# SunJiamei/LRP-ImageCaptioning

Measured on AMD Instinct MI355X. Metric: LRP heatmaps/sec (per predicted token) VGG16+adaptive-attn, 224x224, higher is better.
Workload: dtype bf16x3; 1 GPU; batch=32 synthetic 224x224 per GPU, VGG16 + adaptive-attention, LRP per-token heat-maps, 10 words/caption, V=10000 (BASELINE configs[1]); parallelism=image-sharded x1, RCCL weight broadcast, reverse_walk_precision=bf16x3, handles_per_gpu=2

## Files before the change

include/lrp_hip.h:

```cpp
#ifndef LRP_HIP_H
#define LRP_HIP_H

#include <stddef.h>
#include <stdint.h>

#ifdef __cplusplus
extern "C" {
#endif

#define LRP_ABI_VERSION 10

enum {
  LRP_OK = 0,
  LRP_ERR_INVALID = -1,
  LRP_ERR_STATE = -2,
  LRP_ERR_HIP = -3,
  LRP_ERR_NOMEM = -4,
  LRP_ERR_RANGE = -5,
  LRP_ERR_UNSUPPORTED = -6
};

enum { LRP_DEC_ADAPTIVE = 0,
       LRP_DEC_GRIDTD = 1 };

// ... 148 lines not shown
                   const float* mask_logits_dev, float* grads_dev, float* losses_dev, void* stream);
int lrp_train_forward(lrp_handle* h, int32_t B, int32_t T, const int32_t* cap_in_dev, const float* mask_image_features_dev,
                      const float* mask_global_dev, const float* mask_output_dev, const float* mask_lstm_in_dev,
                      const float* mask_lstm_rec_dev, void* stream);
int lrp_train_drop_forward(lrp_handle* h, void* stream);
int lrp_train_apply(lrp_handle* h, const float* grads_dev, void* stream);
int lrp_train_get_master(lrp_handle* h, float* flat_dev, void* stream);

int64_t lrp_launch_count(void);

int lrp_reload_switches(void);

enum { LRP_EPI_BIAS_RELU = 0, LRP_EPI_BIAS = 1, LRP_EPI_MUL = 2, LRP_EPI_MUL_UP2 = 3, LRP_EPI_FWD_DUAL = 4, LRP_EPI_STORE = 5,
       LRP_EPI_IMG_STENCIL = 6 };
enum { LRP_OPND_FP32 = 0, LRP_OPND_BF16X3 = 1, LRP_OPND_F16X2 = 2 };
enum { LRP_FORM_PLAIN = 0, LRP_FORM_SMALL = 1, LRP_FORM_HALO = 2, LRP_FORM_BREG = 3, LRP_FORM_POOL = 4, LRP_FORM_IMG = 5 };
enum { LRP_PLAN_FRAG = 1, LRP_PLAN_JOIN = 2, LRP_PLAN_DUAL_IL = 4, LRP_PLAN_GMASK = 8,
       LRP_PLAN_UP2_SRC = 16, LRP_PLAN_IMG_PART = 32, LRP_PLAN_POOL_GC = 64 };
int lrp_conv_plan(int32_t epi, int32_t prec, int32_t terms, int32_t NB, int32_t H, int32_t W, int32_t N, int32_t Cin, int32_t taps,
                  int32_t split, uint32_t flags, int32_t* out11);

const char* lrp_last_error(void);
int lrp_abi_version(void);

#ifdef __cplusplus
}
#endif
#endif
```

lrp-imagecaptioning_amd/_capi.py:

```python
import ctypes as C
import os

HERE = os.path.dirname(os.path.abspath(__file__))
LIB_PATH = os.path.join(HERE, "liblrp_hip.so")

LRP_ABI_VERSION = 10
LRP_OK, LRP_ERR_INVALID, LRP_ERR_STATE, LRP_ERR_HIP, LRP_ERR_NOMEM, LRP_ERR_RANGE, LRP_ERR_UNSUPPORTED = 0, -1, -2, -3, -4, -5, -6
LRP_DEC_ADAPTIVE, LRP_DEC_GRIDTD = 0, 1
LRP_ENC_VGG, LRP_ENC_RESNET = 0, 1
LRP_EXPLAIN_SEQUENCE, LRP_EXPLAIN_SINGLE_STEP = 0, 1
LRP_PREC_FP32, LRP_PREC_BF16X3, LRP_PREC_BF16X3_FAST, LRP_PREC_F16X2 = 0, 1, 2, 3
LRP_MAX_CONV = 32
LRP_TRAIN_FP32, LRP_TRAIN_BF16 = 0, 1
LRP_EPI_BIAS_RELU, LRP_EPI_BIAS, LRP_EPI_MUL, LRP_EPI_MUL_UP2, LRP_EPI_FWD_DUAL, LRP_EPI_STORE, LRP_EPI_IMG_STENCIL = range(7)
LRP_OPND_FP32, LRP_OPND_BF16X3, LRP_OPND_F16X2 = 0, 1, 2
LRP_FORM_PLAIN, LRP_FORM_SMALL, LRP_FORM_HALO, LRP_FORM_BREG, LRP_FORM_POOL, LRP_FORM_IMG = range(6)
LRP_PLAN_FRAG, LRP_PLAN_JOIN, LRP_PLAN_DUAL_IL, LRP_PLAN_GMASK, LRP_PLAN_UP2_SRC, LRP_PLAN_IMG_PART, LRP_PLAN_POOL_GC = 1, 2, 4, 8, 16, 32, 64


class LrpConfig(C.Structure):
    _fields_ = [
        ("abi_version", C.c_int32), ("device", C.c_int32), ("decoder", C.c_int32),
        ("img_h", C.c_int32), ("img_w", C.c_int32), ("n_conv", C.c_int32),
        ("conv_cin", C.c_int32 * LRP_MAX_CONV), ("conv_cout", C.c_int32 * LRP_MAX_CONV),
        ("conv_pool_after", C.c_int32 * LRP_MAX_CONV), ("conv_name", (C.c_char * 32) * LRP_MAX_CONV),
        ("L", C.c_int32), ("D", C.c_int32), ("H", C.c_int32), ("E", C.c_int32), ("V", C.c_int32),
        ("max_images", C.c_int32), ("max_tokens", C.c_int32), ("max_caption_len", C.c_int32),
        ("sos_id", C.c_int32), ("eos_id", C.c_int32),
        ("encoder", C.c_int32), ("resnet_stem", C.c_int32), ("resnet_n_stacks", C.c_int32),
        ("resnet_filters", C.c_int32 * 8), ("resnet_blocks", C.c_int32 * 8),
    ]
# ... 102 lines not shown
```

lrp-imagecaptioning_amd/csrc/cnn_kernels.h:

```cpp
#pragma once
#include <hip/hip_runtime.h>
#include "conv_igemm.h"

namespace lrp {

__device__ __forceinline__ float safe_den(float z) { return z + (z == 0.f ? 1e-7f : 0.f); }

__global__ __launch_bounds__(256) void im2col_image_kernel(const float* __restrict__ img, float* __restrict__ A1,
                                                           int NB, int H, int W) {
  const size_t idx = (size_t)blockIdx.x * 256 + threadIdx.x;
  const size_t total = (size_t)NB * H * W * 8;
  if (idx >= total) return;
  const int g = (int)(idx & 7);
  const size_t m = idx >> 3;
  const int HW = H * W;
  const int n = (int)(m / HW), rem = (int)(m - (size_t)n * HW);
  const int h = rem / W, w = rem - h * W;
  const bool neg = g >= 4;
  float v[8];
#pragma unroll
  for (int q = 0; q < 8; ++q) {
    const int kk = 8 * (g & 3) + q;
    float x = 0.f;
    if (kk < 27) {
// ... 390 lines not shown

__global__ __launch_bounds__(256) void pack_image_layer_dev_kernel(const float* __restrict__ w, float* __restrict__ fwd,
                                                                   float* __restrict__ bwd, float* __restrict__ full, int cout, int Kb) {
  const int i = blockIdx.x * 256 + threadIdx.x;
  if (i >= 27 * cout) return;
  const int k = i / cout, co = i - k * cout, t = k / 3, c = k - 3 * t;
  const float v = w[i], vp = v >= 0.f ? v : 0.f, vn = v < 0.f ? v : 0.f;
  fwd[(size_t)co * 64 + k] = v;
  fwd[(size_t)co * 64 + 32 + k] = v;
  fwd[(size_t)(cout + co) * 64 + k] = vp;
  fwd[(size_t)(cout + co) * 64 + 32 + k] = vn;
  bwd[(size_t)(t * 6 + c) * Kb + co] = vp;
  bwd[(size_t)(t * 6 + 3 + c) * Kb + co] = vn;
  full[(size_t)(t * 6 + c) * Kb + co] = v;
}
__global__ __launch_bounds__(256) void pack_frag64_dev_kernel(const float* __restrict__ src, float* __restrict__ dst, int CP) {
  const int K = 9 * CP, cpt = CP / 32;
  const size_t total = (size_t)cpt * 9 * 4 * 2 * 64;
  for (size_t i = (size_t)blockIdx.x * 256 + threadIdx.x; i < total; i += (size_t)gridDim.x * 256) {
    const int n = (int)(i & 63), hh = (int)((i >> 6) & 1), q = (int)((i >> 7) & 3);
    const int kc = (int)(i >> 9), cc = kc / 9, t = kc % 9;
    const int c = 4 * (q >> 1) + 2 * hh + (q & 1);
    *reinterpret_cast<f32x4*>(dst + i * 4) = *reinterpret_cast<const f32x4*>(src + (size_t)n * K + t * CP + cc * 32 + c * 4);
  }
}

__global__ __launch_bounds__(256) void top_divide_kernel(const f32x4* __restrict__ R, const f32x4* __restrict__ Ztop,
                                                         const int* __restrict__ row2img, f32x4* __restrict__ S,
                                                         int n, size_t per_img4) {
  const size_t total = (size_t)n * per_img4;
  for (size_t i = (size_t)blockIdx.x * 256 + threadIdx.x; i < total; i += (size_t)gridDim.x * 256) {
    const int t = (int)(i / per_img4);
    const size_t e = i - (size_t)t * per_img4;
    const int img = row2img ? row2img[t] : t;
    const f32x4 r = R[i], z = Ztop[(size_t)img * per_img4 + e];
    f32x4 o;
// ... 115 lines not shown
```

lrp-imagecaptioning_amd/csrc/common.h:

```cpp
#pragma once
#include <hip/hip_runtime.h>
#include <atomic>
#include <cstdarg>
#include <cstdio>
#include <cstdlib>
#include <string>
#include <vector>

#include "../../include/lrp_hip.h"

namespace lrp {

inline std::atomic<unsigned long long> g_launch_count{0};
#undef hipLaunchKernelGGL
#define hipLaunchKernelGGL(kernelName, numBlocks, numThreads, memPerBlock, streamId, ...)                  \
  do {                                                                                                    \
    ::lrp::g_launch_count.fetch_add(1, std::memory_order_relaxed);                                       \
    kernelName<<<(numBlocks), (numThreads), (memPerBlock), (streamId)>>>(__VA_ARGS__);                   \
  } while (0)

std::string& last_error_ref();

struct Switches {
  int conv_halo = 1;
  int conv_breg = 1;
  int conv_small = 1;
  int conv_mid = 1;
  int epi_fast = 1;
  int up2_pw = 1;
  int tile_order = 1;
  int fwd_emit = 1;
  int fwd_il = 1;
  int img_fused = 1;
  int up2_compact = 1;
  int img_fold = 1;
  int pool_fused = 1;
  int sparse_pool = 1;
  void load() {
    *this = Switches();
    auto rd = [](const char* name, int& v) { if (const char* e = getenv(name)) v = atoi(e); };
    rd("LRP_CONV_HALO", conv_halo); rd("LRP_CONV_BREG", conv_breg); rd("LRP_CONV_SMALL", conv_small);
    rd("LRP_CONV_MID", conv_mid); rd("LRP_EPI_FAST", epi_fast); rd("LRP_UP2_PW", up2_pw); rd("LRP_TILE_ORDER", tile_order);
    rd("LRP_FWD_EMIT", fwd_emit); rd("LRP_FWD_IL", fwd_il); rd("LRP_IMG_FUSED", img_fused); rd("LRP_UP2_COMPACT", up2_compact);
    rd("LRP_IMG_FOLD", img_fold); rd("LRP_SPARSE_POOL", sparse_pool); rd("LRP_POOL_FUSED", pool_fused);
  }
};
inline Switches& sw() {
  static Switches s = [] { Switches t; t.load(); return t; }();
  return s;
}

inline int fail(int code, const char* fmt, ...) {
  char buf[512];
  va_list ap;
  va_start(ap, fmt);
  vsnprintf(buf, sizeof(buf), fmt, ap);
  va_end(ap);
  last_error_ref() = buf;
  return code;
// ... 99 lines not shown
```

lrp-imagecaptioning_amd/csrc/conv_igemm.h:

```cpp
#pragma once
#include <hip/hip_runtime.h>
#include <stdint.h>
#include <stdlib.h>
#include <string.h>
#include <algorithm>
#include <vector>

#include "common.h"

namespace lrp {

typedef float f32x4 __attribute__((ext_vector_type(4)));
typedef float f32x16 __attribute__((ext_vector_type(16)));
typedef unsigned int u32x4 __attribute__((ext_vector_type(4)));
typedef __bf16 bf16x8 __attribute__((ext_vector_type(8)));
typedef _Float16 f16x8 __attribute__((ext_vector_type(8)));

enum ConvPrec { PREC_FP32 = 0, PREC_BF16X3 = 1, PREC_F16X2 = 2 };

__device__ __forceinline__ void split8h_store(const float* r, float* dst) {
  f16x8 hi, lo;
#pragma unroll
  for (int q = 0; q < 8; ++q) {
    hi[q] = (_Float16)r[q];
// ... 98 lines not shown
  float* pool_x;
};
constexpr int ACT_MAX_SLOTS = 64;

constexpr int LDS_STRIDE = 32;

__device__ __attribute__((aligned(16))) float lrp_zero_page[4] = {0.f, 0.f, 0.f, 0.f};

constexpr int conv_min_waves(int NW, int TM, int TN, bool halo = false) { return NW == 8 || halo ? 2 : (TM * TN >= 4 ? 2 : 3); }

constexpr int HALO_PITCH = 16, HALO_PL = 4;
constexpr int conv_halo_rows(int BM) { return BM == 256 ? 352 : 192; }

template <int WM, int WN, int TM, int TN, int EPI, int PREC, bool HALO = false, bool BREG = false, int TERMS = 7, int NS = 2,
          bool GMASK = false>
__global__ __launch_bounds__(64 * WM * WN, BREG ? 3 : NS > 2 ? 2 : conv_min_waves(WM * WN, TM, TN, HALO)) void conv_igemm_kernel(ConvArgs a) {
#if defined(__HIP_DEVICE_COMPILE__)
  constexpr int NW = WM * WN, NT = 64 * NW;
  constexpr bool SPLIT = PREC != PREC_FP32;
  constexpr int BM = WM * TM * 32, BN = WN * TN * 32;
  constexpr int AP = BM / 8 / NW, BP = BN / 8 / NW;
  constexpr int HR = conv_halo_rows(BM);
  constexpr int ABUF = (HALO ? HR : BM) * LDS_STRIDE;
  constexpr int STAGE = ABUF + (BREG ? 0 : BN) * LDS_STRIDE;
  static_assert(!BREG || (HALO && SPLIT && BM * BN <= 2 * STAGE), "BREG needs the resident image");
  static_assert((BM / 8) % NW == 0 && (BN / 8) % NW == 0, "pieces must divide over the waves");
  static_assert(!HALO || EPI != EPI_STORE, "the image layer is a 1-tap GEMM");
  static_assert(NS == 2 || (NS > 2 && !HALO && !BREG), "deeper staging exists for the plain (non-resident) A path only");
  constexpr int DPC = AP + BP;
  static_assert((NS - 2) * DPC <= 63, "vmcnt is a 6-bit counter");
  __shared__ __attribute__((aligned(16))) float smem[NS * STAGE];

  const int nblk = a.m_tiles * a.n_tiles;
  int logical;
  {
    const int bid = blockIdx.x, q = nblk >> 3, r = nblk & 7, xcd = bid & 7, idx = bid >> 3;
    logical = (xcd < r ? xcd * (q + 1) : r * (q + 1) + (xcd - r) * q) + idx;
  }
  const int mt = logical / a.n_tiles, nt = logical - mt * a.n_tiles;
  const int m0 = mt * BM, n0 = nt * BN;
  int pn = 0, py0 = 0, px0 = 0;
  if constexpr (EPI == EPI_IMG_STENCIL) {
    const int tpi = a.tiles_x * a.tiles_y;
    pn = mt / tpi;
    const int r = mt - pn * tpi, ty = r / a.tiles_x;
    py0 = ty * IMG_TILE;
// ... 30 lines not shown
        simg0 = HALO ? img0 : m0 / a.img_rows;
        simg1 = simg0 + 1 < a.n_imgs ? simg0 + 1 : simg0;
      }
      if constexpr (PREC == PREC_F16X2) { us0 = a.in_unscale[simg0]; us1 = a.in_unscale[simg1]; }
      if (a.pairs_out) { ps0 = a.pairs_scale[simg0]; ps1 = a.pairs_scale[simg1]; }
    }
  }

  const int tid = threadIdx.x, lane = tid & 63, wave = tid >> 6;
  const int wm = wave / WN, wn = wave - wm * WN;
  const int HW = a.H * a.W;
  const int K = a.taps * a.CinP;
  const int cpt = a.CinP >> 5;
  const int nk = a.taps * cpt;

  const int prow = lane >> 3, pchk = lane & 7;
  const int wave_s = __builtin_amdgcn_readfirstlane(wave);
  typedef __attribute__((address_space(3))) void* lptr_t;
  constexpr int OOB = (int)0x80000000;
  constexpr int RSRC_FLAGS = 0x00020000;
  const __amdgpu_buffer_rsrc_t rsB =
      __builtin_amdgcn_make_buffer_rsrc((void*)(a.wpk + (size_t)n0 * K), 0, BN * K * 4, RSRC_FLAGS);
  int bvo[BP];
#pragma unroll
  for (int p = 0; p < BP; ++p) {
    const int r = (wave_s * BP + p) * 8 + prow;
    bvo[p] = (r * K + ((pchk ^ ((r >> 1) & 7)) << 2)) * 4;
  }
  const float* abase = HALO ? a.in + (size_t)(Y0 > 0 ? Y0 - 1 : 0) * a.W * a.Cin
                       : EPI == EPI_IMG_STENCIL ? a.in + (size_t)pn * HW * a.Cin
                            : a.in + ((long)m0 - (a.taps == 1 ? 0 : a.W + 1)) * (long)a.Cin;
// ... 156 lines not shown
#pragma unroll
      for (int d = 0; d < 4; ++d) {
        const unsigned p0 = (w.q[d >> 1] >> (16 * (d & 1))) & 0xFFu, p1 = (w.q[d >> 1] >> (16 * (d & 1) + 8)) & 0xFFu;
        const unsigned m = r.valid ? ((p0 == j ? 0x0000FFFFu : 0u) | (p1 == j ? 0xFFFF0000u : 0u)) : 0u;
        mh[d] = w.hi[d] & m;
        ml[d] = w.lo[d] & m;
      }
      const int row = r.hy * HALO_PITCH + hx;
      const int swzu = ((r.hy * a.tw + hx - 1) >> 1) & 7;
      const int dst = abuf * STAGE + row * LDS_STRIDE + (((2 * r.g) ^ swzu) << 2);
      *reinterpret_cast<u32x4*>(smem + dst) = mh;
      *reinterpret_cast<u32x4*>(smem + (dst ^ 4)) = ml;
    }
  };
  [[maybe_unused]] PwItem pwi{};
  if constexpr (BREG) {
    if (PREC == PREC_BF16X3 && a.up2_src) {
      const int Hp = a.H >> 1, Wp = a.W >> 1;
      const int h0 = Y0 - img0 * a.H;
      const int wy0 = (h0 - 1) >> 1, wx0 = (x0 - 1) >> 1;
      const int nwx = ((x0 + a.tw) >> 1) - wx0 + 1, nwy = ((h0 + a.th) >> 1) - wy0 + 1;
      const int items = nwy * nwx * 8;
      const int ntok = img0 < a.NB ? img0 : a.NB - 1;
      const int img = a.row2img ? a.row2img[ntok] : ntok;
      const float inv_nwx = 1.0f / (float)nwx;
      constexpr int UW = 2;
      typedef unsigned u32x2_ __attribute__((ext_vector_type(2)));
      for (int it0 = tid; it0 < items; it0 += NT * UW) {
        f32x4 pv[UW][2];
        u32x2_ qv[UW];
        int wyv[UW], wxv[UW], cgv[UW];
// ... 167 lines not shown
          if constexpr ((TERMS & 2) != 0) acc[i][j] = __builtin_amdgcn_mfma_f32_32x32x16_bf16(ah, bl, acc[i][j], 0, 0, 0);
          if constexpr ((TERMS & 4) != 0) acc[i][j] = __builtin_amdgcn_mfma_f32_32x32x16_bf16(ah, bh, acc[i][j], 0, 0, 0);
        }
    } else {
#pragma unroll
      for (int s = 0; s < 4; ++s)
#pragma unroll
        for (int i = 0; i < TM; ++i)
#pragma unroll
          for (int j = 0; j < TN; ++j)
            acc[i][j] = __builtin_amdgcn_mfma_f32_32x32x2f32(__builtin_bit_cast(f32x4, f.a[i])[s],
                                                             __builtin_bit_cast(f32x4, f.b[j])[s], acc[i][j], 0, 0, 0);
    }
  };

  if constexpr (BREG) {
    static_assert(NSTEP == 2, "bf16x3");
    const __amdgpu_buffer_rsrc_t rsF = __builtin_amdgcn_make_buffer_rsrc((void*)a.wpk_frag, 0, nk * 8 * BN * 16, RSRC_FLAGS);
    const int fvo = ((lane >> 5) * BN + wn * TN * 32 + (lane & 31)) * 16;
    struct BFrag { u32x4 v[4 * TN]; };
    auto load_b = [&](BFrag& b, int kc) {
#pragma unroll
      for (int q = 0; q < 4; q += ((PREC == PREC_F16X2 && !(TERMS & 2)) ? 2 : 1))
#pragma unroll
        for (int j = 0; j < TN; ++j)
          b.v[q * TN + j] = __builtin_amdgcn_raw_buffer_load_b128(rsF, fvo + j * 32 * 16, ((kc * 4 + q) * 2) * BN * 16, 0);
    };
    struct AFrag { u32x4 v[4 * TM]; };
    auto load_a = [&](AFrag& f, const float* Ab) {
#pragma unroll
      for (int q = 0; q < 4; ++q)
// ... 288 lines not shown
        const float sc = a.tok_fac[pn];
#pragma unroll
        for (int c = 0; c < 3; ++c) { pos[c] *= sc; neg[c] *= sc; }
      }
      const float* xv = a.ximg + ((size_t)img * HW + (size_t)y * a.W + x) * 3;
      float* ov = a.out + ((size_t)pn * HW + (size_t)y * a.W + x) * 3;
#pragma unroll
      for (int c = 0; c < 3; ++c) {
        if (a.img_mode == 0) ov[c] = xv[c] >= 0.f ? xv[c] * pos[c] : xv[c] * neg[c];
        else if (a.img_mode == 1) ov[c] = pos[c] + neg[c];
        else ov[c] = xv[c] * (pos[c] + neg[c]);
      }
    }
    return;
  } else if constexpr (EPI != EPI_STORE) {
    constexpr int NH = (BM * BN + 2 * STAGE - 1) / (2 * STAGE);
    constexpr int RH = BM / NH;
    static_assert(BM % NH == 0 && RH % (TM * 32) == 0 && RH * BN <= 2 * STAGE, "slab must hold whole wave tiles");
    float* Cs = smem;
    constexpr bool SPLIT_OUT = SPLIT && (EPI == EPI_MUL || EPI == EPI_MUL_UP2);
    constexpr int CW = SPLIT_OUT ? 8 : 4;
    constexpr int C4 = BN / CW, RPP = NT / C4;
    const int c4 = tid % C4, rin = tid / C4;
    const int col = n0 + c4 * CW;
    const int tn0 = m0 / HW, tp0 = m0 - tn0 * HW;
    const float invw = 1.0f / (float)a.W;
    auto locate = [&](int lr, int& row, int& n, int& h, int& w) -> bool {
      if constexpr (HALO) {
        int ty, tx;
        divmod(lr, a.tw, inv_tw, ty, tx);
        const int Y = Y0 + ty;
        w = x0 + tx;
        if (lr >= a.th * a.tw || Y >= yend || w >= a.W) return false;
// ... 527 lines not shown
struct ConvTile { int BM, BN; };
inline ConvTile conv_pick_tile(int N) {
  if (N > 64) return {128, 128};
  if (N > 32) return {128, 64};
  return {128, 32};
}
inline int conv_npad(int N) { ConvTile t = conv_pick_tile(N); return (N + t.BN - 1) / t.BN * t.BN; }
inline int conv_cinp(int Cin) { return (Cin + 31) / 32 * 32; }

enum ConvForm {
  FORM_PLAIN = 0,
  FORM_SMALL = 1,
  FORM_HALO = 2,
  FORM_BREG = 3,
  FORM_POOL = 4,
  FORM_IMG = 5
};
struct ConvAsk {
  int epi = EPI_MUL, prec = PREC_FP32, terms = 7;
  bool gmask = false;
  int NB = 0, H = 0, W = 0, N = 0, Cin = 0, taps = 9;
  bool frag = false;
  bool join = false;
  bool dual_il = false;
  int split = 0;
  bool up2_src = false, img_part = false, pool_gc = false;
};
struct ConvPlan {
  bool ok;
  int form, BM, BN, threads;
  int M, m_tiles, n_tiles, tw, th, hrows, cols_t, nyh, tpt, epi_generic;
// ... 95 lines not shown
  const bool small = s.conv_small && t.BM == 128 && t.BN >= 64 && grid <= CONV_SMALL_BLOCKS;
  if (q.up2_src) {
    if (!mul || prec != PREC_BF16X3 || !s.up2_pw || mode <= 0 || t.BN < 128 || small || !conv_compact_shape(q.N, q.Cin, q.H, q.W))
      return refused;
  } else if (small) {
    t = {64, 64};
    p.m_tiles = (p.M + 63) / 64;
    p.n_tiles = (q.N + 63) / 64;
    return done(FORM_SMALL);
  } else if (s.conv_mid && s.conv_small && t.BM == 128 && t.BN == 128 && (q.N % 64) == 0 && grid <= 2 * CONV_SMALL_BLOCKS) {
    t = {128, 64};
    p.n_tiles = (q.N + 63) / 64;
  }
  if (mode > 0 && (t.BN >= 128 || (mode == 2 && t.BN >= 64)) && resident(false, 0.9f)) {
    if (q.up2_src && p.hrows * ((p.tw + 2) / 2 + 1) * 4 > 2 * (t.BM == 256 ? 512 : 256)) return refused;
    return done(FORM_HALO);
  }
  if (asked) return refused;
  return done(FORM_PLAIN);
}

inline const int* conv_tile_order(const ConvArgs& a, hipStream_t st) {
  if (!sw().tile_order || !a.order || !a.row2img_host || a.NB < 2 || a.th < 1) return nullptr;
  TileOrder& o = *a.order;
  const int tiles_y = a.tpt > 0 ? a.NB * a.tpt : (a.nyh + a.th - 1) / a.th;
  const bool same = o.H == a.H && o.th == a.th && o.nyh == a.nyh && o.cols_t == a.cols_t && o.tpt == a.tpt && (int)o.sig.size() == a.NB &&
                    memcmp(o.sig.data(), a.row2img_host, (size_t)a.NB * sizeof(int)) == 0;
  if (same) return o.identity ? nullptr : o.dev;
  o.sig.assign(a.row2img_host, a.row2img_host + a.NB);
  o.H = a.H; o.th = a.th; o.nyh = a.nyh; o.cols_t = a.cols_t; o.tpt = a.tpt;
// ... 81 lines not shown
inline hipError_t conv_launch_epi(ConvArgs a, hipStream_t st) {
  static_assert(!GMASK || (EPI == EPI_MUL && PREC == PREC_FP32), "byte-mask gates: exact fp32 EPI_MUL only");
  constexpr bool MUL = EPI == EPI_MUL || EPI == EPI_MUL_UP2, FWD = EPI == EPI_BIAS || EPI == EPI_BIAS_RELU || EPI == EPI_FWD_DUAL;
  if (GMASK && (a.out2s || a.gate_none)) return hipErrorInvalidValue;
  if (PREC == PREC_F16X2 && MUL && (!a.tok_fac || !a.tok_max_out || a.out_plain)) return hipErrorInvalidValue;
  if (PREC == PREC_F16X2 && FWD && !a.in_unscale) return hipErrorInvalidValue;
  const ConvPlan p = conv_plan(conv_ask(EPI, PREC, TERMS, GMASK, a));
  if (!p.ok) return hipErrorInvalidValue;
  if (p.M <= 0 || a.N <= 0) return hipSuccess;
  if (a.pool_gc && (!a.pairs_out || !a.pool_pos)) return hipErrorInvalidValue;
  if (a.img_part && !a.img_w) return hipErrorInvalidValue;
  if (a.up2_src && (!a.up2_pairs || !a.up2_gpos)) return hipErrorInvalidValue;
  conv_apply_plan(p, a);
  const dim3 grid(p.m_tiles * p.n_tiles), block(p.threads);
  if constexpr (PREC != PREC_FP32 && (MUL || FWD)) {
    if (p.form == FORM_BREG || p.form == FORM_HALO || p.form == FORM_POOL) {
      if constexpr (MUL) {
        a.tile_map = conv_tile_order(a, st);
        if (p.form == FORM_BREG) {
          hipLaunchKernelGGL((conv_igemm_kernel<2, 2, 2, 1, EPI, PREC, true, true, TERMS>), grid, block, 0, st, a);
          return hipGetLastError();
        }
      }
      if (p.BM == 256)
        hipLaunchKernelGGL((conv_igemm_kernel<2, 4, 4, 2, EPI, PREC, true, false, TERMS>), grid, block, 0, st, a);
      else if (p.BN == 128)
        hipLaunchKernelGGL((conv_igemm_kernel<2, 2, 2, 2, EPI, PREC, true, false, TERMS>), grid, block, 0, st, a);
      else
        hipLaunchKernelGGL((conv_igemm_kernel<2, 2, 2, 1, EPI, PREC, true, false, TERMS>), grid, block, 0, st, a);
      return hipGetLastError();
    }
  }
  if constexpr (PREC != PREC_FP32) {
// ... 69 lines not shown
```

lrp-imagecaptioning_amd/csrc/encoder.h:

```cpp
#pragma once
#include <algorithm>
#include <functional>
#include <memory>
#include <string>
#include <vector>

#include "cnn_kernels.h"
#include "common.h"
#include "conv_igemm.h"
#include "conv_sparse.h"
#include "f16_operand.h"
#include "fwd_mode.h"

namespace lrp {

struct ConvLayer {
  std::string name;
  int cin = 0, cout = 0, H = 0, W = 0;
  bool pool_after = false;
  bool have_w = false, have_b = false;
  DevBuf w_fwd;
  DevBuf w_fwd_a;
  DevBuf w_fwd_zs;
  DevBuf w_fwd_as;
// ... 188 lines not shown
        L.w_fwd_il.release();
      }
      LRP_TRY(mk(L.w_bwd, nb)); LRP_TRY(mk(L.w_bwd_s, nb)); LRP_TRY(mk(L.w_bwd_full, nb)); LRP_TRY(mk(L.w_bwd_h, nb));
      return LRP_OK;
    }
    const size_t Kf = (size_t)9 * conv_cinp(L.cin), Kb = (size_t)9 * conv_cinp(L.cout);
    const size_t nf = (size_t)conv_npad(L.cout) * Kf, nb = (size_t)conv_npad(L.cin) * Kb;
    LRP_TRY(mk(L.w_fwd, (size_t)conv_npad(2 * L.cout) * Kf)); LRP_TRY(mk(L.w_fwd_h, (size_t)conv_npad(2 * L.cout) * Kf));
    if (dual_interleaved(L)) LRP_TRY(mk(L.w_fwd_il, (size_t)conv_npad(2 * L.cout) * Kf));
    else L.w_fwd_il.release();
    LRP_TRY(mk(L.w_fwd_a, nf)); LRP_TRY(mk(L.w_fwd_zs, nf)); LRP_TRY(mk(L.w_fwd_as, nf));
    LRP_TRY(mk(L.w_bwd, nb)); LRP_TRY(mk(L.w_bwd_s, nb)); LRP_TRY(mk(L.w_bwd_full, nb)); LRP_TRY(mk(L.w_bwd_full_s, nb));
    LRP_TRY(mk(L.w_bwd_h, nb));
    if (L.sparse_ok() && L.idxp.p) LRP_TRY(mk(L.w_sp, conv_sparse_weight_floats(L.cin, L.cout)));
    if (conv_npad(L.cin) == 64) { LRP_TRY(mk(L.w_bwd_frag, (size_t)64 * Kb)); LRP_TRY(mk(L.w_bwd_frag_h, (size_t)64 * Kb)); }
    if (pack_tmp.bytes < nf * sizeof(float)) LRP_TRY(pack_tmp.alloc(nf * sizeof(float), total));
    return LRP_OK;
  }
  int repack_conv_weight_from_device(int li, const float* w_dev, float* tmp, hipStream_t st) {
    ConvLayer& L = layers[li];
    if (li == 0) {
      const int Npb = conv_npad(IMG_T_COLS), Kb = conv_cinp(L.cout);
      hipLaunchKernelGGL(pack_image_layer_dev_kernel, dim3((27 * L.cout + 255) / 256), dim3(256), 0, st, w_dev, L.w_fwd.as<float>(),
                         L.w_bwd.as<float>(), L.w_bwd_full.as<float>(), L.cout, Kb);
      const size_t nb = (size_t)Npb * Kb;
      if (L.w_fwd_il.p) {
        hipLaunchKernelGGL(dual_interleave_rows_kernel, dim3(stream_grid((size_t)2 * L.cout * 64)), dim3(256), 0, st, L.w_fwd.as<float>(),
                           L.w_fwd_il.as<float>(), L.cout, 64);
        LRP_TRY(make_f16_operand(L.w_fwd_il.as<float>(), (size_t)conv_npad(2 * L.cout) * 64, 0, 0, L.w_fwd_h, L.wds, nullptr, st));
      }
// ... 13 lines not shown
      hipLaunchKernelGGL(split_copy_kernel, dim3(stream_grid(n / 8)), dim3(256), 0, st, src, dst, n / 8);
    };
    const size_t nf = (size_t)Npa * 9 * CPi, nb = (size_t)Npb * 9 * CPo;
    pack(L.w_fwd.as<float>(), 0, Np2, 1, 0);
    if (L.w_fwd_il.p) pack(L.w_fwd_il.as<float>(), 0, Np2, 2, 0);
    LRP_TRY(make_f16_operand(L.w_fwd_il.p ? L.w_fwd_il.as<float>() : L.w_fwd.as<float>(), (size_t)Np2 * 9 * CPi, 0, 0, L.w_fwd_h,
                             L.wds, nullptr, st));
    pack(L.w_fwd_a.as<float>(), 0, Npa, 0, 0);
    pack(tmp, 0, Npa, 0, 1);
    split(tmp, L.w_fwd_zs.as<float>(), nf);
    split(L.w_fwd_a.as<float>(), L.w_fwd_as.as<float>(), nf);
    pack(L.w_bwd.as<float>(), 1, Npb, 0, 1);
    split(L.w_bwd.as<float>(), L.w_bwd_s.as<float>(), nb);
    if (L.w_sp.p) LRP_HIP_CHECK(conv_sparse_pack(L.w_bwd.as<float>(), L.w_sp.as<float>(), L.cin, L.cout, st));
    if (L.w_bwd_frag.p)
      hipLaunchKernelGGL(pack_frag64_dev_kernel, dim3(stream_grid((size_t)CPo / 32 * 9 * 512)), dim3(256), 0, st, L.w_bwd_s.as<float>(),
                         L.w_bwd_frag.as<float>(), CPo);
    LRP_TRY(make_f16_operand(L.w_bwd.as<float>(), nb, Npb, 9 * CPo, L.w_bwd_h, L.wbs, nullptr, st));
    if (L.w_bwd_frag_h.p)
      hipLaunchKernelGGL(pack_frag64_dev_kernel, dim3(stream_grid((size_t)CPo / 32 * 9 * 512)), dim3(256), 0, st, L.w_bwd_h.as<float>(),
                         L.w_bwd_frag_h.as<float>(), CPo);
    pack(L.w_bwd_full.as<float>(), 1, Npb, 0, 0);
    split(L.w_bwd_full.as<float>(), L.w_bwd_full_s.as<float>(), nb);
    LRP_HIP_CHECK(hipGetLastError());
    return LRP_OK;
  }
  int repack_conv_from_device(int li, const float* w_dev, const float* b_dev, float* tmp, hipStream_t st) {
    ConvLayer& L = layers[li];
    if (!L.have_w || !L.have_b) return fail(LRP_ERR_STATE, "layer %d has no operand copies to rebuild", li);
    LRP_TRY(repack_conv_weight_from_device(li, w_dev, tmp, st));
    L.norm_dirty = true;
    LRP_HIP_CHECK(hipMemcpyAsync(L.bias.p, b_dev, (size_t)L.cout * sizeof(float), hipMemcpyDeviceToDevice, st));
    L.raw_w_dev.release(); L.raw_b_dev.release();
    return LRP_OK;
  }
  int set_conv_weight_dev(int li, const float* w, hipMemcpyKind kind, int64_t* total, hipStream_t st) {
// ... 519 lines not shown
```

lrp-imagecaptioning_amd/csrc/engine.hip:

```cpp
#include <hip/hip_runtime.h>

#include <cmath>
#include <cstring>
#include <exception>
#include <map>
#include <new>
#include <string>
#include <vector>

#include "common.h"
#include "conv_igemm.h"
#include "conv_sparse.h"
#include "decoder.h"
#include "encoder.h"
#include "eval_kernels.h"
#include "gradcam_kernels.h"
#include "perturb_kernels.h"
#include "resnet_encoder.h"
#include "rules_kernels.h"
#include "score_kernels.h"
#include "trainer.h"

namespace lrp {
std::string& last_error_ref() {
// ... 71 lines not shown
extern "C" {

int lrp_abi_version(void) { return LRP_ABI_VERSION; }
int lrp_reload_switches(void) {
  return guarded([&]() -> int { lrp::sw().load(); return LRP_OK; });
}

int lrp_conv_plan(int32_t epi, int32_t prec, int32_t terms, int32_t NB, int32_t H, int32_t W, int32_t N, int32_t Cin, int32_t taps,
                  int32_t split, uint32_t flags, int32_t* out11) {
  return guarded([&]() -> int {
    static_assert(LRP_EPI_BIAS_RELU == lrp::EPI_BIAS_RELU && LRP_EPI_BIAS == lrp::EPI_BIAS && LRP_EPI_MUL == lrp::EPI_MUL &&
                  LRP_EPI_MUL_UP2 == lrp::EPI_MUL_UP2 && LRP_EPI_FWD_DUAL == lrp::EPI_FWD_DUAL && LRP_EPI_STORE == lrp::EPI_STORE &&
                  LRP_EPI_IMG_STENCIL == lrp::EPI_IMG_STENCIL, "lrp_hip.h LRP_EPI_*");
    static_assert(LRP_OPND_FP32 == lrp::PREC_FP32 && LRP_OPND_BF16X3 == lrp::PREC_BF16X3 && LRP_OPND_F16X2 == lrp::PREC_F16X2, "lrp_hip.h LRP_OPND_*");
    static_assert(LRP_FORM_PLAIN == lrp::FORM_PLAIN && LRP_FORM_SMALL == lrp::FORM_SMALL && LRP_FORM_HALO == lrp::FORM_HALO &&
                  LRP_FORM_BREG == lrp::FORM_BREG && LRP_FORM_POOL == lrp::FORM_POOL && LRP_FORM_IMG == lrp::FORM_IMG, "lrp_hip.h LRP_FORM_*");
    if (!out11) return fail(LRP_ERR_INVALID, "null argument");
    lrp::ConvAsk q;
    q.epi = epi; q.prec = prec; q.terms = terms; q.NB = NB; q.H = H; q.W = W; q.N = N; q.Cin = Cin; q.taps = taps; q.split = split;
    q.frag = flags & LRP_PLAN_FRAG; q.join = flags & LRP_PLAN_JOIN; q.dual_il = flags & LRP_PLAN_DUAL_IL; q.gmask = flags & LRP_PLAN_GMASK;
    q.up2_src = flags & LRP_PLAN_UP2_SRC; q.img_part = flags & LRP_PLAN_IMG_PART; q.pool_gc = flags & LRP_PLAN_POOL_GC;
    const lrp::ConvPlan p = lrp::conv_plan(q);
    const int v[11] = {p.ok ? 1 : 0, p.form, p.BM, p.BN, p.threads, p.tw, p.th, p.hrows, p.tpt, p.m_tiles, p.n_tiles};
    for (int i = 0; i < 11; ++i) out11[i] = v[i];
    return LRP_OK;
  });
}

int64_t lrp_launch_count(void) { return (int64_t)lrp::g_launch_count.load(std::memory_order_relaxed); }
const char* lrp_last_error(void) { return last_error_ref().c_str(); }

// ... 319 lines not shown
    mode &= ~LRP_CONV_SPLIT_BF16;
    if (mode < 0 || mode > 3) return fail(LRP_ERR_INVALID, "mode must be 0..3");
    if (split && mode == 0) return fail(LRP_ERR_UNSUPPORTED, "the split-bf16 path has no relu epilogue (modes 1..3)");
    const bool bwd = mode >= 2;
    const int inC = bwd ? Cout : Cin, outC = bwd ? Cin : Cout;
    if (inC % 4 != 0) return fail(LRP_ERR_UNSUPPORTED, "input channels must be a multiple of 4");
    if (split && ((inC & 7) || (bwd && (outC & 7)))) return fail(LRP_ERR_UNSUPPORTED, "split-bf16 path: channels must be multiples of 8");
    const int Np = conv_npad(outC), K = taps * conv_cinp(inC);
    hipStream_t st = S(stream);
    DevBuf wraw, wdev, wsplit, bdev, insplit, wfrag;
    LRP_TRY(op_pack_weight(w_hwio_host, taps, Cin, Cout, bwd, wraw, wdev, st));
    if (split) {
      const size_t nw8 = (size_t)Np * K / 8;
      LRP_TRY(wsplit.alloc(wdev.bytes, nullptr));
      hipLaunchKernelGGL(split_copy_kernel, dim3(stream_grid(nw8)), dim3(256), 0, st, wdev.as<float>(), wsplit.as<float>(), nw8);
      if (bwd && taps == 9 && Np == 64) {
        LRP_TRY(wfrag.alloc((size_t)64 * K * sizeof(float), nullptr));
        hipLaunchKernelGGL(pack_frag64_dev_kernel, dim3(stream_grid((size_t)conv_cinp(inC) / 32 * 9 * 512)), dim3(256), 0, st,
                           wsplit.as<float>(), wfrag.as<float>(), conv_cinp(inC));
      }
      const size_t n8 = (size_t)NB * H * W * inC / 8;
      LRP_TRY(insplit.alloc(n8 * 32, nullptr));
      hipLaunchKernelGGL(split_copy_kernel, dim3(stream_grid(n8)), dim3(256), 0, st, in_dev, insplit.as<float>(), n8);
      LRP_HIP_CHECK(hipGetLastError());
      in_dev = insplit.as<float>();
    }
    ConvArgs ca{};
    ca.out_plain = 1;
    ca.wpk_frag = wfrag.as<float>();
    ca.in = in_dev; ca.wpk = split ? wsplit.as<float>() : wdev.as<float>(); ca.NB = NB; ca.H = H; ca.W = W; ca.Cin = inC; ca.CinP = conv_cinp(inC);
    ca.N = outC; ca.taps = taps; ca.out = out_dev; ca.aux = aux_dev;
    if (!bwd) {
      if (!bias_host) return fail(LRP_ERR_INVALID, "bias required for forward modes");
      LRP_TRY(bdev.alloc((size_t)Cout * sizeof(float), nullptr));
// ... 495 lines not shown
```

Before: 10030 heatmaps/s.

## Add 8-wave register-resident weight-fragment conv form for bf16x3 backward walk

Adds a new FORM_BREG8 conv variant: an 8-wave (2x4) kernel that streams pre-packed weight fragments straight into registers with triple buffering, holding only the double-buffered halo image in LDS. The planner selects it for BM=256 bf16x3 EPI_MUL backward layers that were previously handled by the HALO form. The weight fragment packer is generalised to any row count, and fragments are now built for layers with Cin divisible by 256. The aim is to cut LDS traffic for B and raise MFMA density on the large VGG backward convs. The cost is extra fragment memory and a lower occupancy bound.

```diff
diff --git a/include/lrp_hip.h b/include/lrp_hip.h
--- a/include/lrp_hip.h
+++ b/include/lrp_hip.h
@@ -186,7 +186,7 @@
 enum { LRP_EPI_BIAS_RELU = 0, LRP_EPI_BIAS = 1, LRP_EPI_MUL = 2, LRP_EPI_MUL_UP2 = 3, LRP_EPI_FWD_DUAL = 4, LRP_EPI_STORE = 5,
        LRP_EPI_IMG_STENCIL = 6 };
 enum { LRP_OPND_FP32 = 0, LRP_OPND_BF16X3 = 1, LRP_OPND_F16X2 = 2 };
-enum { LRP_FORM_PLAIN = 0, LRP_FORM_SMALL = 1, LRP_FORM_HALO = 2, LRP_FORM_BREG = 3, LRP_FORM_POOL = 4, LRP_FORM_IMG = 5 };
+enum { LRP_FORM_PLAIN = 0, LRP_FORM_SMALL = 1, LRP_FORM_HALO = 2, LRP_FORM_BREG = 3, LRP_FORM_POOL = 4, LRP_FORM_IMG = 5, LRP_FORM_BREG8 = 6 };
 enum { LRP_PLAN_FRAG = 1, LRP_PLAN_JOIN = 2, LRP_PLAN_DUAL_IL = 4, LRP_PLAN_GMASK = 8,
        LRP_PLAN_UP2_SRC = 16, LRP_PLAN_IMG_PART = 32, LRP_PLAN_POOL_GC = 64 };
 int lrp_conv_plan(int32_t epi, int32_t prec, int32_t terms, int32_t NB, int32_t H, int32_t W, int32_t N, int32_t Cin, int32_t taps,
diff --git a/lrp-imagecaptioning_amd/_capi.py b/lrp-imagecaptioning_amd/_capi.py
--- a/lrp-imagecaptioning_amd/_capi.py
+++ b/lrp-imagecaptioning_amd/_capi.py
@@ -14,7 +14,7 @@
 LRP_TRAIN_FP32, LRP_TRAIN_BF16 = 0, 1
 LRP_EPI_BIAS_RELU, LRP_EPI_BIAS, LRP_EPI_MUL, LRP_EPI_MUL_UP2, LRP_EPI_FWD_DUAL, LRP_EPI_STORE, LRP_EPI_IMG_STENCIL = range(7)
 LRP_OPND_FP32, LRP_OPND_BF16X3, LRP_OPND_F16X2 = 0, 1, 2
-LRP_FORM_PLAIN, LRP_FORM_SMALL, LRP_FORM_HALO, LRP_FORM_BREG, LRP_FORM_POOL, LRP_FORM_IMG = range(6)
+LRP_FORM_PLAIN, LRP_FORM_SMALL, LRP_FORM_HALO, LRP_FORM_BREG, LRP_FORM_POOL, LRP_FORM_IMG, LRP_FORM_BREG8 = range(7)
 LRP_PLAN_FRAG, LRP_PLAN_JOIN, LRP_PLAN_DUAL_IL, LRP_PLAN_GMASK, LRP_PLAN_UP2_SRC, LRP_PLAN_IMG_PART, LRP_PLAN_POOL_GC = 1, 2, 4, 8, 16, 32, 64
 
 
diff --git a/lrp-imagecaptioning_amd/csrc/cnn_kernels.h b/lrp-imagecaptioning_amd/csrc/cnn_kernels.h
--- a/lrp-imagecaptioning_amd/csrc/cnn_kernels.h
+++ b/lrp-imagecaptioning_amd/csrc/cnn_kernels.h
@@ -428,12 +428,13 @@
   bwd[(size_t)(t * 6 + 3 + c) * Kb + co] = vn;
   full[(size_t)(t * 6 + c) * Kb + co] = v;
 }
-__global__ __launch_bounds__(256) void pack_frag64_dev_kernel(const float* __restrict__ src, float* __restrict__ dst, int CP) {
+__global__ __launch_bounds__(256) void pack_frag_dev_kernel(const float* __restrict__ src, float* __restrict__ dst, int CP, int rows) {
   const int K = 9 * CP, cpt = CP / 32;
-  const size_t total = (size_t)cpt * 9 * 4 * 2 * 64;
-  for (size_t i = (size_t)blockIdx.x * 256 + threadIdx.x; i < total; i += (size_t)gridDim.x * 256) {
-    const int n = (int)(i & 63), hh = (int)((i >> 6) & 1), q = (int)((i >> 7) & 3);
-    const int kc = (int)(i >> 9), cc = kc / 9, t = kc % 9;
+  const size_t total = (size_t)cpt * 9 * 4 * 2 * rows;
+  for (size_t i = (size_t)blockIdx.x * 256 + threadIdx.x; i < total; i += (size_t)gridDim.x * 256) {
+    const size_t f = i / rows;
+    const int n = (int)(i - f * rows), hh = (int)(f & 1), q = (int)((f >> 1) & 3);
+    const int kc = (int)(f >> 3), cc = kc / 9, t = kc % 9;
     const int c = 4 * (q >> 1) + 2 * hh + (q & 1);
     *reinterpret_cast<f32x4*>(dst + i * 4) = *reinterpret_cast<const f32x4*>(src + (size_t)n * K + t * CP + cc * 32 + c * 4);
   }
diff --git a/lrp-imagecaptioning_amd/csrc/common.h b/lrp-imagecaptioning_amd/csrc/common.h
--- a/lrp-imagecaptioning_amd/csrc/common.h
+++ b/lrp-imagecaptioning_amd/csrc/common.h
@@ -24,6 +24,7 @@
 struct Switches {
   int conv_halo = 1;
   int conv_breg = 1;
+  int conv_breg8 = 1;
   int conv_small = 1;
   int conv_mid = 1;
   int epi_fast = 1;
@@ -43,6 +44,7 @@
     rd("LRP_CONV_MID", conv_mid); rd("LRP_EPI_FAST", epi_fast); rd("LRP_UP2_PW", up2_pw); rd("LRP_TILE_ORDER", tile_order);
     rd("LRP_FWD_EMIT", fwd_emit); rd("LRP_FWD_IL", fwd_il); rd("LRP_IMG_FUSED", img_fused); rd("LRP_UP2_COMPACT", up2_compact);
     rd("LRP_IMG_FOLD", img_fold); rd("LRP_SPARSE_POOL", sparse_pool); rd("LRP_POOL_FUSED", pool_fused);
+    if (const char* e = getenv("LRP_CONV_BREG8")) conv_breg8 = atoi(e);
   }
 };
 inline Switches& sw() {
diff --git a/lrp-imagecaptioning_amd/csrc/conv_igemm.h b/lrp-imagecaptioning_amd/csrc/conv_igemm.h
--- a/lrp-imagecaptioning_amd/csrc/conv_igemm.h
+++ b/lrp-imagecaptioning_amd/csrc/conv_igemm.h
@@ -136,7 +136,7 @@
 
 template <int WM, int WN, int TM, int TN, int EPI, int PREC, bool HALO = false, bool BREG = false, int TERMS = 7, int NS = 2,
           bool GMASK = false>
-__global__ __launch_bounds__(64 * WM * WN, BREG ? 3 : NS > 2 ? 2 : conv_min_waves(WM * WN, TM, TN, HALO)) void conv_igemm_kernel(ConvArgs a) {
+__global__ __launch_bounds__(64 * WM * WN, BREG && WM * WN != 8 ? 3 : NS > 2 ? 2 : conv_min_waves(WM * WN, TM, TN, HALO)) void conv_igemm_kernel(ConvArgs a) {
 #if defined(__HIP_DEVICE_COMPILE__)
   constexpr int NW = WM * WN, NT = 64 * NW;
   constexpr bool SPLIT = PREC != PREC_FP32;
@@ -145,13 +145,17 @@
   constexpr int HR = conv_halo_rows(BM);
   constexpr int ABUF = (HALO ? HR : BM) * LDS_STRIDE;
   constexpr int STAGE = ABUF + (BREG ? 0 : BN) * LDS_STRIDE;
-  static_assert(!BREG || (HALO && SPLIT && BM * BN <= 2 * STAGE), "BREG needs the resident image");
+  constexpr bool BREG8 = BREG && NW == 8;
+  static_assert(!BREG || (HALO && SPLIT && (BREG8 || BM * BN <= 2 * STAGE)), "BREG needs the resident image");
+  static_assert(!BREG8 || (PREC == PREC_BF16X3 && EPI == EPI_MUL && TERMS == 7 && TM == 4 && TN == 2), "one instantiation: the dense split-bf16 walk");
   static_assert((BM / 8) % NW == 0 && (BN / 8) % NW == 0, "pieces must divide over the waves");
   static_assert(!HALO || EPI != EPI_STORE, "the image layer is a 1-tap GEMM");
   static_assert(NS == 2 || (NS > 2 && !HALO && !BREG), "deeper staging exists for the plain (non-resident) A path only");
   constexpr int DPC = AP + BP;
   static_assert((NS - 2) * DPC <= 63, "vmcnt is a 6-bit counter");
-  __shared__ __attribute__((aligned(16))) float smem[NS * STAGE];
+  constexpr int SMEM = BREG8 ? (2 * STAGE > BM / 2 * BN ? 2 * STAGE : BM / 2 * BN) : NS * STAGE;
+  constexpr int CSLAB = BREG8 ? SMEM : 2 * STAGE;
+  __shared__ __attribute__((aligned(16))) float smem[SMEM];
 
   const int nblk = a.m_tiles * a.n_tiles;
   int logical;
@@ -212,7 +216,7 @@
   const int cpt = a.CinP >> 5;
   const int nk = a.taps * cpt;
 
-  const int prow = lane >> 3, pchk = lane & 7;
+  int prow = lane >> 3, pchk = lane & 7;
   const int wave_s = __builtin_amdgcn_readfirstlane(wave);
   typedef __attribute__((address_space(3))) void* lptr_t;
   constexpr int OOB = (int)0x80000000;
@@ -399,7 +403,9 @@
     }
   };
   [[maybe_unused]] PwItem pwi{};
-  if constexpr (BREG) {
+  if constexpr (BREG8) {
+    for (int p = wave_s; p < halo_np; p += NW) fire_halo_piece(prep_halo_piece(p, 0, true), p, 0);
+  } else if constexpr (BREG) {
     if (PREC == PREC_BF16X3 && a.up2_src) {
       const int Hp = a.H >> 1, Wp = a.W >> 1;
       const int h0 = Y0 - img0 * a.H;
@@ -597,7 +603,71 @@
     }
   };
 
-  if constexpr (BREG) {
+  if constexpr (BREG8) {
+    static_assert(NSTEP == 2 && SMEM >= 2 * STAGE + NW * 8 * LDS_STRIDE, "bf16x3; a spare LDS slot per wave behind the two images");
+    const int NF = a.n_tiles * BN;
+    const int nsteps = 2 * nk;
+    const __amdgpu_buffer_rsrc_t rsF = __builtin_amdgcn_make_buffer_rsrc((void*)a.wpk_frag, 0, nsteps * 4 * NF * 16, RSRC_FLAGS);
+    const int fvo = ((lane >> 5) * NF + n0 + wn * TN * 32 + (lane & 31)) * 16;
+    u32x4 bq[3][2 * TN];
+    u32x4 aq[2 * TM];
+    auto load_b = [&](u32x4* b, int gs) {
+      const int so = (gs < nsteps ? gs : nsteps - 1) * 4 * NF * 16;
+#pragma unroll
+      for (int hl = 0; hl < 2; ++hl)
+#pragma unroll
+        for (int j = 0; j < TN; ++j)
+          b[hl * TN + j] = __builtin_amdgcn_raw_buffer_load_b128(rsF, fvo + j * 32 * 16, so + hl * 2 * NF * 16, 0);
+    };
+    load_b(bq[0], 0);
+    load_b(bq[1], 1);
+    set_tap(0);
+#pragma unroll
+    for (int i = 0; i < TM; ++i) {
+      aq[2 * i] = *reinterpret_cast<const u32x4*>(smem + faddr[i]);
+      aq[2 * i + 1] = *reinterpret_cast<const u32x4*>(smem + (faddr[i] ^ 4));
+    }
+    for (int c = 0; c < cpt; ++c) {
+      const int cb = c & 1;
+      const float* Ab = smem + cb * STAGE;
+      const float* An = smem + (cb ^ 1) * STAGE;
+#pragma unroll
+      for (int i = 0; i < TM; ++i) asm volatile("" : "+v"(fbase[i]), "+v"(fu[i]));
+      asm volatile("" : "+v"(prow), "+v"(pchk));
+#pragma unroll
+      for (int s = 0; s < 18; ++s) {
+        load_b(bq[(s + 2) % 3], c * 18 + s + 2);
+        if (s % 3 == 0) {
+          const int p = (s / 3) * NW + wave_s;
+          const bool livep = p < halo_np;
+          const HaloPiece hp = prep_halo_piece(p, c + 1, livep && c + 1 < cpt);
+          const int dst = livep ? (cb ^ 1) * STAGE + p * 8 * LDS_STRIDE : 2 * STAGE + wave_s * 8 * LDS_STRIDE;
+          __builtin_amdgcn_raw_ptr_buffer_load_lds(rsA, (lptr_t)(smem + dst), 16, hp.vo, hp.so, 0, 0);
+        }
+        if (s == 17) {
+          asm volatile("s_waitcnt vmcnt(8) lgkmcnt(0)\n\ts_barrier" ::: "memory");
+        }
+        const int nst = (s + 1) & 1;
+        if (nst == 0) set_tap(((s + 1) >> 1) % 9);
+        const float* Ax = s == 17 ? An : Ab;
+        __builtin_amdgcn_sched_barrier(0);
+#pragma unroll
+        for (int i = 0; i < TM; ++i) {
+          const bf16x8 ah = __builtin_bit_cast(bf16x8, aq[2 * i]), al = __builtin_bit_cast(bf16x8, aq[2 * i + 1]);
+#pragma unroll
+          for (int j = 0; j < TN; ++j) {
+            const bf16x8 bh = __builtin_bit_cast(bf16x8, bq[s % 3][j]), bl = __builtin_bit_cast(bf16x8, bq[s % 3][TN + j]);
+            acc[i][j] = __builtin_amdgcn_mfma_f32_32x32x16_bf16(al, bh, acc[i][j], 0, 0, 0);
+            acc[i][j] = __builtin_amdgcn_mfma_f32_32x32x16_bf16(ah, bl, acc[i][j], 0, 0, 0);
+            acc[i][j] = __builtin_amdgcn_mfma_f32_32x32x16_bf16(ah, bh, acc[i][j], 0, 0, 0);
+          }
+          aq[2 * i] = *reinterpret_cast<const u32x4*>(Ax + (faddr[i] ^ ((4 * nst) << 2)));
+          aq[2 * i + 1] = *reinterpret_cast<const u32x4*>(Ax + (faddr[i] ^ ((4 * nst + 1) << 2)));
+          __builtin_amdgcn_sched_barrier(0);
+        }
+      }
+    }
+  } else if constexpr (BREG) {
     static_assert(NSTEP == 2, "bf16x3");
     const __amdgpu_buffer_rsrc_t rsF = __builtin_amdgcn_make_buffer_rsrc((void*)a.wpk_frag, 0, nk * 8 * BN * 16, RSRC_FLAGS);
     const int fvo = ((lane >> 5) * BN + wn * TN * 32 + (lane & 31)) * 16;
@@ -916,9 +986,9 @@
     }
     return;
   } else if constexpr (EPI != EPI_STORE) {
-    constexpr int NH = (BM * BN + 2 * STAGE - 1) / (2 * STAGE);
+    constexpr int NH = (BM * BN + CSLAB - 1) / CSLAB;
     constexpr int RH = BM / NH;
-    static_assert(BM % NH == 0 && RH % (TM * 32) == 0 && RH * BN <= 2 * STAGE, "slab must hold whole wave tiles");
+    static_assert(BM % NH == 0 && RH % (TM * 32) == 0 && RH * BN <= CSLAB, "slab must hold whole wave tiles");
     float* Cs = smem;
     constexpr bool SPLIT_OUT = SPLIT && (EPI == EPI_MUL || EPI == EPI_MUL_UP2);
     constexpr int CW = SPLIT_OUT ? 8 : 4;
@@ -1476,7 +1546,8 @@
   FORM_HALO = 2,
   FORM_BREG = 3,
   FORM_POOL = 4,
-  FORM_IMG = 5
+  FORM_IMG = 5,
+  FORM_BREG8 = 6
 };
 struct ConvAsk {
   int epi = EPI_MUL, prec = PREC_FP32, terms = 7;
@@ -1602,6 +1673,8 @@
   }
   if (mode > 0 && (t.BN >= 128 || (mode == 2 && t.BN >= 64)) && resident(false, 0.9f)) {
     if (q.up2_src && p.hrows * ((p.tw + 2) / 2 + 1) * 4 > 2 * (t.BM == 256 ? 512 : 256)) return refused;
+    if (s.conv_breg8 && t.BM == 256 && prec == PREC_BF16X3 && epi == EPI_MUL && q.terms == 7 && q.frag && !asked && !q.join)
+      return done(FORM_BREG8);
     return done(FORM_HALO);
   }
   if (asked) return refused;
@@ -1713,9 +1786,16 @@
   conv_apply_plan(p, a);
   const dim3 grid(p.m_tiles * p.n_tiles), block(p.threads);
   if constexpr (PREC != PREC_FP32 && (MUL || FWD)) {
-    if (p.form == FORM_BREG || p.form == FORM_HALO || p.form == FORM_POOL) {
+    if (p.form == FORM_BREG || p.form == FORM_HALO || p.form == FORM_POOL || p.form == FORM_BREG8) {
       if constexpr (MUL) {
         a.tile_map = conv_tile_order(a, st);
+        if constexpr (EPI == EPI_MUL && PREC == PREC_BF16X3 && TERMS == 7) {
+          if (p.form == FORM_BREG8) {
+            hipLaunchKernelGGL((conv_igemm_kernel<2, 4, 4, 2, EPI_MUL, PREC_BF16X3, true, true, 7>), grid, block, 0, st, a);
+            return hipGetLastError();
+          }
+        }
+        if (p.form == FORM_BREG8) return hipErrorInvalidValue;
         if (p.form == FORM_BREG) {
           hipLaunchKernelGGL((conv_igemm_kernel<2, 2, 2, 1, EPI, PREC, true, true, TERMS>), grid, block, 0, st, a);
           return hipGetLastError();
diff --git a/lrp-imagecaptioning_amd/csrc/encoder.h b/lrp-imagecaptioning_amd/csrc/encoder.h
--- a/lrp-imagecaptioning_amd/csrc/encoder.h
+++ b/lrp-imagecaptioning_amd/csrc/encoder.h
@@ -226,6 +226,7 @@
     LRP_TRY(mk(L.w_bwd_h, nb));
     if (L.sparse_ok() && L.idxp.p) LRP_TRY(mk(L.w_sp, conv_sparse_weight_floats(L.cin, L.cout)));
     if (conv_npad(L.cin) == 64) { LRP_TRY(mk(L.w_bwd_frag, (size_t)64 * Kb)); LRP_TRY(mk(L.w_bwd_frag_h, (size_t)64 * Kb)); }
+    else if (sw().conv_breg8 && (L.cin % 256) == 0 && !(L.cout & 7)) LRP_TRY(mk(L.w_bwd_frag, nb));
     if (pack_tmp.bytes < nf * sizeof(float)) LRP_TRY(pack_tmp.alloc(nf * sizeof(float), total));
     return LRP_OK;
   }
@@ -269,12 +270,12 @@
     split(L.w_bwd.as<float>(), L.w_bwd_s.as<float>(), nb);
     if (L.w_sp.p) LRP_HIP_CHECK(conv_sparse_pack(L.w_bwd.as<float>(), L.w_sp.as<float>(), L.cin, L.cout, st));
     if (L.w_bwd_frag.p)
-      hipLaunchKernelGGL(pack_frag64_dev_kernel, dim3(stream_grid((size_t)CPo / 32 * 9 * 512)), dim3(256), 0, st, L.w_bwd_s.as<float>(),
-                         L.w_bwd_frag.as<float>(), CPo);
+      hipLaunchKernelGGL(pack_frag_dev_kernel, dim3(stream_grid((size_t)CPo / 32 * 9 * 8 * Npb)), dim3(256), 0, st, L.w_bwd_s.as<float>(),
+                         L.w_bwd_frag.as<float>(), CPo, Npb);
     LRP_TRY(make_f16_operand(L.w_bwd.as<float>(), nb, Npb, 9 * CPo, L.w_bwd_h, L.wbs, nullptr, st));
     if (L.w_bwd_frag_h.p)
-      hipLaunchKernelGGL(pack_frag64_dev_kernel, dim3(stream_grid((size_t)CPo / 32 * 9 * 512)), dim3(256), 0, st, L.w_bwd_h.as<float>(),
-                         L.w_bwd_frag_h.as<float>(), CPo);
+      hipLaunchKernelGGL(pack_frag_dev_kernel, dim3(stream_grid((size_t)CPo / 32 * 9 * 512)), dim3(256), 0, st, L.w_bwd_h.as<float>(),
+                         L.w_bwd_frag_h.as<float>(), CPo, 64);
     pack(L.w_bwd_full.as<float>(), 1, Npb, 0, 0);
     split(L.w_bwd_full.as<float>(), L.w_bwd_full_s.as<float>(), nb);
     LRP_HIP_CHECK(hipGetLastError());
diff --git a/lrp-imagecaptioning_amd/csrc/engine.hip b/lrp-imagecaptioning_amd/csrc/engine.hip
--- a/lrp-imagecaptioning_amd/csrc/engine.hip
+++ b/lrp-imagecaptioning_amd/csrc/engine.hip
@@ -109,7 +109,7 @@
                   LRP_EPI_IMG_STENCIL == lrp::EPI_IMG_STENCIL, "lrp_hip.h LRP_EPI_*");
     static_assert(LRP_OPND_FP32 == lrp::PREC_FP32 && LRP_OPND_BF16X3 == lrp::PREC_BF16X3 && LRP_OPND_F16X2 == lrp::PREC_F16X2, "lrp_hip.h LRP_OPND_*");
     static_assert(LRP_FORM_PLAIN == lrp::FORM_PLAIN && LRP_FORM_SMALL == lrp::FORM_SMALL && LRP_FORM_HALO == lrp::FORM_HALO &&
-                  LRP_FORM_BREG == lrp::FORM_BREG && LRP_FORM_POOL == lrp::FORM_POOL && LRP_FORM_IMG == lrp::FORM_IMG, "lrp_hip.h LRP_FORM_*");
+                  LRP_FORM_BREG == lrp::FORM_BREG && LRP_FORM_POOL == lrp::FORM_POOL && LRP_FORM_IMG == lrp::FORM_IMG && LRP_FORM_BREG8 == lrp::FORM_BREG8, "lrp_hip.h LRP_FORM_*");
     if (!out11) return fail(LRP_ERR_INVALID, "null argument");
     lrp::ConvAsk q;
     q.epi = epi; q.prec = prec; q.terms = terms; q.NB = NB; q.H = H; q.W = W; q.N = N; q.Cin = Cin; q.taps = taps; q.split = split;
@@ -459,10 +459,10 @@
       const size_t nw8 = (size_t)Np * K / 8;
       LRP_TRY(wsplit.alloc(wdev.bytes, nullptr));
       hipLaunchKernelGGL(split_copy_kernel, dim3(stream_grid(nw8)), dim3(256), 0, st, wdev.as<float>(), wsplit.as<float>(), nw8);
-      if (bwd && taps == 9 && Np == 64) {
-        LRP_TRY(wfrag.alloc((size_t)64 * K * sizeof(float), nullptr));
-        hipLaunchKernelGGL(pack_frag64_dev_kernel, dim3(stream_grid((size_t)conv_cinp(inC) / 32 * 9 * 512)), dim3(256), 0, st,
-                           wsplit.as<float>(), wfrag.as<float>(), conv_cinp(inC));
+      if (bwd && taps == 9 && (Np == 64 || (sw().conv_breg8 && (outC % 256) == 0))) {
+        LRP_TRY(wfrag.alloc((size_t)Np * K * sizeof(float), nullptr));
+        hipLaunchKernelGGL(pack_frag_dev_kernel, dim3(stream_grid((size_t)conv_cinp(inC) / 32 * 9 * 8 * Np)), dim3(256), 0, st,
+                           wsplit.as<float>(), wfrag.as<float>(), conv_cinp(inC), Np);
       }
       const size_t n8 = (size_t)NB * H * W * inC / 8;
       LRP_TRY(insplit.alloc(n8 * 32, nullptr));
diff --git a/profiles/walk_regweights_ab.py b/profiles/walk_regweights_ab.py
--- /dev/null
+++ b/profiles/walk_regweights_ab.py
@@ -0,0 +1,52 @@
+#!/usr/bin/env python3
+import os, sys, statistics
+import numpy as np
+sys.path.insert(0, os.path.dirname(os.path.dirname(os.path.abspath(__file__))))
+PASSES = int(sys.argv[1]) if len(sys.argv) > 1 else 5
+import torch
+from bench import synth_weights
+from lrp_imagecaptioning_amd.engine import LRPEngine, switches
+from lrp_imagecaptioning_amd.synthetic import VGG16_CFG, captions, images
+B, T, V = 32, 10, 10000
+eng = LRPEngine(decoder="adaptive", V=V, max_images=B, max_tokens=B * T, max_caption_len=T + 1)
+eng.set_weights(synth_weights(0, V))
+rs = np.random.RandomState(1)
+X = torch.as_tensor(images(rs, B)).cuda()
+caps = captions(rs, B, T, V)
+idx = [b for b in range(B) for _ in range(T)]
+tpos = [t for _ in range(B) for t in range(1, T + 1)]
+out = torch.empty((B * T, 224, 224, 3), dtype=torch.float32, device="cuda")
+eng.encode_images(X); eng.decoder_forward(caps)
+ref = {}
+for on in (1, 0):
+    with switches(LRP_CONV_BREG8=on):
+        eng.explain_tokens(idx, tpos, out=out); torch.cuda.synchronize()
+        ref[on] = out.clone()
+print("heat-maps bit-identical on/off:", bool(torch.equal(ref[0], ref[1])), "finite:", bool(torch.isfinite(ref[1]).all()), flush=True)
+names = [c[0] for c in VGG16_CFG][::-1]
+res = {0: [], 1: []}
+for p in range(PASSES):
+    for on in (0, 1):
+        with switches(LRP_CONV_BREG8=on):
+            eng.explain_tokens(idx, tpos, out=out); torch.cuda.synchronize()
+            eng.profile_enable(True)
+            acc = None
+            for _ in range(3):
+                eng.explain_tokens(idx, tpos, out=out); torch.cuda.synchronize()
+                rec = eng.profile_records()
+                acc = rec if acc is None else [(a + b, f) for (a, f), (b, _) in zip(acc, rec)]
+            eng.profile_enable(False)
+            res[on].append([m / 3 for m, _ in acc])
+        print("pass %d BREG8=%d walk %.3f ms: %s" % (p, on, sum(res[on][-1]), " ".join("%.3f" % m for m in res[on][-1])), flush=True)
+print("records per walk:", len(res[0][0]), names[:len(res[0][0])])
+print("%-14s %28s %28s" % ("layer", "BREG8=0 med [min,max]", "BREG8=1 med [min,max]"))
+for k in range(len(res[0][0])):
+    row = []
+    for on in (0, 1):
+        v = [r[k] for r in res[on]]
+        row.append("%.3f [%.3f, %.3f]" % (statistics.median(v), min(v), max(v)))
+    won = statistics.median([r[k] for r in res[1]]) < min(r[k] for r in res[0])
+    print("%-14s %28s %28s %s" % (names[k] if k < len(names) else k, row[0], row[1], "WON" if won else ""))
+for on in (0, 1):
+    v = [sum(r) for r in res[on]]
+    print("walk total BREG8=%d: %.3f [%.3f, %.3f]" % (on, statistics.median(v), min(v), max(v)))
```

Result: faster. 10460 heatmaps/s (median of 6 runs) (+4.3%).
